# zhoujoey/ORB-SLAM3-Mac

Measured on AMD Instinct MI355X. Metric: ORB extract+match frames/sec, higher is better.
Workload: dtype u8; 1 GPU; vga: synthetic 640x480 batch=1024 per GPU, 8-level pyramid, 1000 feats/frame, ORB extract + Hamming 2-NN match (Frame.cc:1146) + SearchForInitialization (ORBmatcher.cc:710) vs successor frame; pipelines=1, matchers=side by side (two contexts), frames_total=1024

## Files before the change

### orb-slam3-mac_amd/csrc/orb_internal.h

```cpp
#pragma once
#include <hip/hip_runtime.h>
#include <stdint.h>
#include "../../include/orbhip.h"

#define ORB_MAX_LEVELS 16
#define ORB_EDGE 19
#define ORB_MINB 16
#define ORB_HALF_PATCH 15
#define ORB_RS_STEPS 24

struct OrbLevel {
    uint8_t *img;
    uint8_t *blur;
    size_t img_frame_stride;
    size_t blur_frame_stride;
    int w, h, img_pitch, blur_pitch;
    int ncols, nrows, wcell, hcell;
    int cell_base;
    int cell_cap;
    int quota;
    int key_base, key_cap;
    int kp_base, kp_cap;
    int n_ini;
    float hx;
    float scale;
    float size;
    const int16_t *xofs; const int16_t *xalpha; const int16_t *yofs; const int16_t *ybeta;
    const uint32_t *xchunk; const uint32_t *ytab;
    int resize_mode;
    int rs_rows;
};

struct OrbParams {
    OrbLevel lv[ORB_MAX_LEVELS];
    int nlevels, batch;
    int n_cus;
    int ini_th, min_th;
    int cells_per_frame;
    int keys_per_frame;
    int kps_per_frame;
    int max_kp;
    int oct_nc;
    int rows_min_batch;
    int bm_min_batch;
    int br_blocks[ORB_MAX_LEVELS + 1];
    int bs_tiles[ORB_MAX_LEVELS + 1];
    int lap0, lap1;
    uint32_t *cell_count;
    uint32_t *cell_list;
    size_t cell_list_frame_stride;
    uint32_t *keys;
    uint16_t *node_of;
    uint32_t *lvl_kp;
#define ORB_PERM_MIN_BATCH 16
    uint16_t *lvl_perm;
    float *lvl_angle;
    uint8_t *lvl_desc;
    int32_t *lvl_count;
    int32_t *lvl_ncand;
    int32_t *status;
    orbhip_keypoint *out_kp;
    uint8_t *out_desc;
    int32_t *out_count;
    int32_t *out_mono;
    int umax[ORB_HALF_PATCH + 1];
// ... 43 lines not shown
struct StereoArgs {
    StereoLevel lv[ORB_MAX_LEVELS];
    int nlevels, batch, max_kp, rows0;
    const orbhip_keypoint *kpL, *kpR;
    const uint8_t *descL, *descR;
    const int32_t *nL, *nR;
    float mb, mbf;
    float *u_right, *depth;
    int32_t *sad, *n_kept;
};
void orb_launch_stereo(const StereoArgs &A, hipStream_t s);

int orb_lds_optin(const void *func, int device, size_t need);

void orb_launch_resize(const OrbParams &P, int level, hipStream_t s);
void orb_launch_fast_cells(const FastParams &F, hipStream_t s, int max_per_cu, int lvl_lo = 0, int lvl_hi = -1);
const void *orb_fast_runs_func(int nld);
#define ORB_OVERLAP_MIN_BATCH 16
#ifndef BLR_R
#define BLR_R 24
#endif
void orb_launch_blur(const OrbParams &P, hipStream_t s, int wgs_per_cu, int frame0 = 0, int nframes = -1);
const void *orb_fast_cells_func(int small);
void orb_launch_octree(const OrbParams &P, hipStream_t s);
void orb_launch_orient_desc(const OrbParams &P, hipStream_t s);
void orb_launch_assemble(const OrbParams &P, hipStream_t s);
size_t orb_octree_lds_bytes(int nc);
int orb_octree_nc(const OrbParams &P);
const void *orb_octree_func();
```

### orb-slam3-mac_amd/csrc/orb_kernels.hip

```cpp
#include "orb_internal.h"
#include "wave_dpp.h"
#include <mutex>
#include <vector>
#include <cstdio>
#include <cstdlib>

#define WAVE 64

__device__ __forceinline__ int wave_incl_scan(int v) { return wave_scan_add_dpp(v); }

__device__ __forceinline__ int block_excl_scan256(int v, int *wsum, int *total)
{
    const int lane = threadIdx.x & (WAVE - 1), wid = threadIdx.x >> 6;
    int inc = wave_incl_scan(v);
    if (lane == WAVE - 1) wsum[wid] = inc;
    __syncthreads();
    int base = 0;
#pragma unroll
    for (int w = 0; w < 4; w++) {
        int s = wsum[w];
        if (w < wid) base += s;
    }
    *total = wsum[0] + wsum[1] + wsum[2] + wsum[3];
    __syncthreads();
// ... 784 lines not shown
}

__device__ __forceinline__ int oct_quadrant(uint32_t key, uint32_t b0, uint32_t b1)
{
    const int x0 = b0 & 0xFFFF, y0 = b0 >> 16, x1 = b1 & 0xFFFF, y1 = b1 >> 16;
    const int mx = x0 + ((x1 - x0 + 1) >> 1), my = y0 + ((y1 - y0 + 1) >> 1);
    const int kx = ORB_KEY_X(key), ky = ORB_KEY_Y(key);
    return (kx < mx ? 0 : 1) + (ky < my ? 0 : 2);
}

#define OCT_KR 8
#ifdef OCT_PROF
__device__ long long g_oct_prof[8];
#define OCT_T(i) do { if (blockIdx.x == 0 && threadIdx.x == 0) { const long long t_ = clock64(); g_oct_prof[i] += t_ - t_prev; t_prev = t_; } } while (0)
extern "C" int orbhip_debug_oct_prof(long long *out8, int reset)
{
    if (out8 && hipMemcpyFromSymbol(out8, HIP_SYMBOL(g_oct_prof), 64) != hipSuccess) return -1;
    if (reset) { long long z[8] = {0}; if (hipMemcpyToSymbol(HIP_SYMBOL(g_oct_prof), z, 64) != hipSuccess) return -1; }
    return 0;
}
#else
#define OCT_T(i) do { } while (0)
#endif
__global__ __launch_bounds__(256) void k_octree(OrbParams P)
{
    extern __shared__ uint32_t smem[];
    __shared__ int wsum[8];
    __shared__ int s_size, s_front, s_nexpand, s_rstar, s_T, s_nproc;
    const int tid = threadIdx.x;
#ifdef OCT_PROF
    long long t_prev = clock64();
#endif
    const int lvl = blockIdx.x / P.batch;
    const int frame = blockIdx.x - lvl * P.batch;
    const OrbLevel &L = P.lv[lvl];
    const int N = L.quota;
    const int NC = P.oct_nc;
    uint32_t *box0 = smem, *box1 = smem + NC, *cnt = smem + 2 * NC;
    uint32_t *nbox0 = smem + 3 * NC, *nbox1 = smem + 4 * NC, *ncnt = smem + 5 * NC;
    OctLds S;
    {
        uint32_t *p = smem + 6 * NC;
        S.cc = p; p += 4 * NC;
        S.ord = (int *)p; p += NC; S.by_ord = (int *)p; p += NC; S.excl = (int *)p; p += NC;
        S.posbase = (int *)p; p += NC; S.newpos = (int *)p; p += NC; S.best = p; p += NC;
    }
    const uint32_t *ccount = P.cell_count + (size_t)frame * P.cells_per_frame + L.cell_base;
    const uint32_t *clist = P.cell_list + (size_t)frame * P.cell_list_frame_stride + (size_t)L.cell_base * L.cell_cap;
    uint32_t *keys = P.keys + (size_t)frame * P.keys_per_frame + L.key_base;
    uint16_t *node_of = P.node_of + (size_t)frame * P.keys_per_frame + L.key_base;
    const int ncells = L.ncols * L.nrows;
    uint32_t rk[OCT_KR]; int rn[OCT_KR];
    int running = 0;
    int32_t *count_out = P.lvl_count + frame * P.nlevels + lvl;
    if (ncells + 1 <= 16 * NC) {
        int *coff = reinterpret_cast<int *>(smem);
        for (int c0 = 0; c0 < ncells; c0 += 256) {
            const int c = c0 + tid;
            const int n = c < ncells ? min((int)ccount[c], L.cell_cap) : 0;
            int total;
            const int off = running + block_excl_scan256(n, wsum, &total);
            if (c < ncells) coff[c] = off;
            running += total;
        }
        if (tid == 0) coff[ncells] = running;
        __syncthreads();
        if (running > L.key_cap) { if (tid == 0) atomicExch(P.status, ORBHIP_E_CAPACITY); running = L.key_cap; }
        const int K0 = running;
        auto fetch = [&](int k) {
            int lo = 0, hi = ncells;
            while (hi - lo > 1) { const int mid = (lo + hi) >> 1; if (coff[mid] <= k) lo = mid; else hi = mid; }
            return clist[(size_t)lo * L.cell_cap + (k - coff[lo])];
        };
#pragma unroll
        for (int i = 0; i < OCT_KR; i++) { const int k = tid + 256 * i; rk[i] = k < K0 ? fetch(k) : 0u; rn[i] = 0; }
#pragma unroll
        for (int i = 0; i < OCT_KR; i++) { const int k = tid + 256 * i; if (k < K0) keys[k] = rk[i]; }
        for (int k = tid + 256 * OCT_KR; k < K0; k += 256) keys[k] = fetch(k);
        __syncthreads();
    } else {
        for (int c0 = 0; c0 < ncells; c0 += 256) {
            const int c = c0 + tid;
            const int n = c < ncells ? (int)ccount[c] : 0;
            int total;
            const int off = running + block_excl_scan256(n, wsum, &total);
            for (int i = 0; i < n; i++)
                if (off + i < L.key_cap) keys[off + i] = clist[(size_t)c * L.cell_cap + i];
            running += total;
        }
        if (running > L.key_cap) { if (tid == 0) atomicExch(P.status, ORBHIP_E_CAPACITY); running = L.key_cap; }
        __syncthreads();
        __threadfence_block();
#pragma unroll
        for (int i = 0; i < OCT_KR; i++) { const int k = tid + 256 * i; rk[i] = k < running ? keys[k] : 0u; rn[i] = 0; }
    }
    const int K = running;
    if (tid == 0) P.lvl_ncand[frame * P.nlevels + lvl] = K;
    if (K == 0) { if (tid == 0) *count_out = 0; return; }
    __syncthreads();
    __threadfence_block();
    OCT_T(0);
    const int n_ini = L.n_ini;
    const int H = (L.h - ORB_MINB) - ORB_MINB;
    for (int i = tid; i < NC; i += 256) { cnt[i] = 0; ncnt[i] = 0; }
    __syncthreads();
#pragma unroll
    for (int i = 0; i < OCT_KR; i++)
        if (tid + 256 * i < K) {
            const int r = (int)__fdiv_rn((float)ORB_KEY_X(rk[i]), L.hx);
            rn[i] = r;
            atomicAdd(&ncnt[r], 1u);
        }
    for (int k = tid + 256 * OCT_KR; k < K; k += 256) {
        const int r = (int)__fdiv_rn((float)ORB_KEY_X(keys[k]), L.hx);
        node_of[k] = (uint16_t)r;
        atomicAdd(&ncnt[r], 1u);
    }
    __syncthreads();
    if (tid == 0) {
        int m = 0;
// ... 143 lines not shown
                int r = 0;
                for (int j = 3; j > qd; j--) r += q[j] > 0;
                return S.posbase[p] + r;
            }
            return S.newpos[p];
        };
#pragma unroll
        for (int i = 0; i < OCT_KR; i++) if (tid + 256 * i < K) rn[i] = relabel(rk[i], rn[i]);
        for (int k = tid + 256 * OCT_KR; k < K; k += 256) node_of[k] = (uint16_t)relabel(keys[k], node_of[k]);
        __syncthreads();
        const int new_size = T + (size - nproc);
        const int nexpand = s_nexpand;
        { uint32_t *t; t = box0; box0 = nbox0; nbox0 = t; t = box1; box1 = nbox1; nbox1 = t; t = cnt; cnt = ncnt; ncnt = t; }
        const int old_size = size;
        size = new_size; front = T;
#ifdef OCT_PROF
        if (blockIdx.x == 0 && tid == 0) g_oct_prof[5] += 1;
#endif
        if (new_size >= N || new_size == old_size) break;
        if (!final_phase && new_size + 3 * nexpand > N) final_phase = true;
    }
    __syncthreads();
    OCT_T(2);
    for (int i = tid; i < size; i += 256) S.best[i] = 0;
    __syncthreads();
#pragma unroll
    for (int i = 0; i < OCT_KR; i++)
        if (tid + 256 * i < K) atomicMax(&S.best[rn[i]], ((uint32_t)ORB_KEY_S(rk[i]) << 20) | (uint32_t)(0xFFFFF - (tid + 256 * i)));
    for (int k = tid + 256 * OCT_KR; k < K; k += 256)
        atomicMax(&S.best[node_of[k]], ((uint32_t)ORB_KEY_S(keys[k]) << 20) | (uint32_t)(0xFFFFF - k));
    __syncthreads();
    OCT_T(3);
    uint32_t *out = P.lvl_kp + (size_t)frame * P.kps_per_frame + L.kp_base;
    int nout = size;
    if (nout > L.kp_cap) { if (tid == 0) atomicExch(P.status, ORBHIP_E_CAPACITY); nout = L.kp_cap; }
    uint16_t *perm = P.lvl_perm + (size_t)frame * P.kps_per_frame + L.kp_base;
    for (int i = tid; i < nout; i += 256) out[i] = keys[0xFFFFF - (S.best[i] & 0xFFFFF)];
    if (P.batch < ORB_PERM_MIN_BATCH) { if (tid == 0) *count_out = nout; return; }
    __syncthreads();
    for (int i = tid; i < nout; i += 256) { const uint32_t ki = out[i]; S.best[i] = ((uint32_t)(ORB_KEY_Y(ki) >> 5) << 16) | (uint32_t)ORB_KEY_X(ki); }
    __syncthreads();
    for (int i = tid; i < nout; i += 256) {
        const uint32_t si = S.best[i];
        int rank = 0;
        for (int j = 0; j < nout; j++) { const uint32_t sj = S.best[j]; rank += (sj < si) || (sj == si && j < i); }
        perm[rank] = (uint16_t)i;
    }
    if (tid == 0) *count_out = nout;
    OCT_T(4);
}

const void *orb_octree_func() { return reinterpret_cast<const void *>(k_octree); }

void orb_launch_octree(const OrbParams &P, hipStream_t s)
{
    const size_t lds = orb_octree_lds_bytes(P.oct_nc);
    hipLaunchKernelGGL(k_octree, dim3(P.nlevels * P.batch), dim3(256), lds, s, P);
}

#define BL_TW 64
#define BL_TH 32
#define BL_ROWS (BL_TH + 6)
#define BL_IPD 20
__device__ __forceinline__ int reflect101(int p, int n)
{
    if (p < 0) p = -p;
    if (p >= n) p = 2 * n - 2 - p;
    return p;
}

__device__ __forceinline__ uint32_t bl_load4(const uint8_t *row, int x, int w)
{
    if (x >= 0 && x + 3 < w) return *reinterpret_cast<const uint32_t *>(row + x);
    uint32_t v = 0;
#pragma unroll
    for (int j = 0; j < 4; j++) {
        int xx = reflect101(x + j, w);
        xx = min(max(xx, 0), w - 1);
        v |= (uint32_t)row[xx] << (8 * j);
    }
// ... 579 lines not shown
```

### orb-slam3-mac_amd/csrc/orbhip_api.hip

```cpp
#include "orb_internal.h"
#include "ctx_internal.h"
#include <cmath>
#include <cfloat>
#include <cstdio>
#include <cstdlib>
#include <cstring>
#include <string>
#include <vector>
#include <mutex>
#include <set>
#include <utility>

static thread_local std::string g_last_error;
extern "C" const char *orbhip_last_error(void) { return g_last_error.c_str(); }
extern "C" const char *orbhip_version(void) { return "orbhip 0.1 (gfx950)"; }

#define HIP_TRY(expr)                                                                   \
    do {                                                                                \
        hipError_t _e = (expr);                                                         \
        if (_e != hipSuccess) {                                                         \
            g_last_error = std::string(#expr) + ": " + hipGetErrorString(_e);           \
            return ORBHIP_E_HIP;                                                        \
        }                                                                               \
    } while (0)
// ... 185 lines not shown
    int width, height, max_batch;
    bool level0_owned;
    OrbParams P;
    FastParams F;
    std::vector<void *> allocs;
    size_t bytes_reserved;
    int last_batch;
    bool profiling;
    hipEvent_t ev[ORBHIP_PROF_SLOTS][ORBHIP_STAGE_COUNT + 1];
    int ev_calls;
    bool ev_created;
    float stage_ms[ORBHIP_STAGE_COUNT];
    uint8_t *d_level0;
    int32_t *d_stereo_sad;
    bool graph_mode, graph_valid;
    hipStream_t aux; hipEvent_t ev_fork, ev_join, ev_pyr; bool aux_ok; int overlap;
    hipGraphExec_t graph_exec;
    int g_w, g_h, g_batch, g_lap0, g_lap1;
    size_t level0_frame_stride; int level0_pitch;
    uint8_t *d_outblob; size_t outblob_bytes, ob_kp, ob_desc;
    uint8_t *h_out; uint8_t *h_in; size_t h_in_bytes; int32_t *h_status;
    uint8_t *h_pyr; size_t h_pyr_bytes;
    unsigned long long generation, view_generation;
};

extern "C" int orbhip_extractor_create(orbhip_ctx *ctx, int nfeatures, float scale_factor, int nlevels,
                                       int ini_th, int min_th, orbhip_extractor **out)
{
    if (!ctx || !out || nlevels < 1 || nlevels > ORB_MAX_LEVELS || nfeatures < 1 || !(scale_factor > 1.0f) || scale_factor > 2.0f)
        return ORBHIP_E_BADARG;
    orbhip_extractor *e = new orbhip_extractor();
    e->ctx = ctx; e->nfeatures = nfeatures; e->nlevels = nlevels; e->ini_th = ini_th; e->min_th = min_th;
    e->scale_factor = scale_factor;
    e->width = e->height = e->max_batch = 0; e->bytes_reserved = 0; e->last_batch = 0;
    e->profiling = false; e->ev_created = false; e->ev_calls = 0; e->d_level0 = nullptr; e->level0_owned = false;
    e->d_stereo_sad = nullptr;
    e->graph_mode = false; e->graph_valid = false; e->graph_exec = nullptr;
    e->aux = nullptr; e->ev_fork = e->ev_join = e->ev_pyr = nullptr; e->aux_ok = false; e->overlap = 1;
    e->d_outblob = nullptr; e->outblob_bytes = e->ob_kp = e->ob_desc = 0; e->h_out = e->h_in = e->h_pyr = nullptr; e->h_in_bytes = e->h_pyr_bytes = 0; e->h_status = nullptr;
    e->generation = 0; e->view_generation = ~0ull;
    memset(&e->P, 0, sizeof(e->P));
    memset(e->stage_ms, 0, sizeof(e->stage_ms));
    e->scale[0] = 1.0f; e->sigma2[0] = 1.0f;
    for (int i = 1; i < nlevels; i++) { e->scale[i] = e->scale[i - 1] * scale_factor; e->sigma2[i] = e->scale[i] * e->scale[i]; }
    for (int i = 0; i < nlevels; i++) { e->inv_scale[i] = 1.0f / e->scale[i]; e->inv_sigma2[i] = 1.0f / e->sigma2[i]; }
    float factor = 1.0f / scale_factor;
// ... 338 lines not shown
    }
    if ((rc = dev_alloc(e, &P.cell_count, B * cells))) return rc;
    if ((rc = dev_alloc(e, &P.cell_list, B * P.cell_list_frame_stride))) return rc;
    if ((rc = dev_alloc(e, &P.keys, B * keys))) return rc;
    if ((rc = dev_alloc(e, &P.node_of, B * keys))) return rc;
    if ((rc = dev_alloc(e, &P.lvl_kp, B * kps))) return rc;
    if ((rc = dev_alloc(e, &P.lvl_perm, B * kps))) return rc;
    if ((rc = dev_alloc(e, &P.lvl_angle, B * kps))) return rc;
    if ((rc = dev_alloc(e, &P.lvl_desc, B * kps * 32))) return rc;
    if ((rc = dev_alloc(e, &P.lvl_count, B * e->nlevels))) return rc;
    if ((rc = dev_alloc(e, &P.lvl_ncand, B * e->nlevels))) return rc;
    if ((rc = dev_alloc(e, &P.status, 1))) return rc;
    {
        auto up = [](size_t v) { return (v + 255) & ~(size_t)255; };
        e->ob_kp = up(8 * B); e->ob_desc = e->ob_kp + up(sizeof(orbhip_keypoint) * B * P.max_kp);
        e->outblob_bytes = e->ob_desc + up((size_t)32 * B * P.max_kp);
        if ((rc = dev_alloc(e, &e->d_outblob, e->outblob_bytes))) return rc;
        P.out_count = reinterpret_cast<int32_t *>(e->d_outblob); P.out_mono = P.out_count + B;
        P.out_kp = reinterpret_cast<orbhip_keypoint *>(e->d_outblob + e->ob_kp); P.out_desc = e->d_outblob + e->ob_desc;
    }
    HIP_TRY(hipMemset(P.status, 0, sizeof(int32_t)));
    P.oct_nc = orb_octree_nc(P);
    if (orb_octree_lds_bytes(P.oct_nc) > 150 * 1024) { g_last_error = "per-level quota (or nIni) too large for the LDS-resident octree"; return ORBHIP_E_BADARG; }
    if ((rc = orb_lds_optin(orb_octree_func(), e->ctx->device, orb_octree_lds_bytes(P.oct_nc)))) return rc;
    if ((rc = orb_lds_optin(orb_fast_cells_func(e->F.small_cells), e->ctx->device, sizeof(uint32_t) * (size_t)e->F.wave_dw))) return rc;
    if (e->F.use_runs && (rc = orb_lds_optin(orb_fast_runs_func((e->F.run_rows - 7) * 5 <= 256 ? 4 : 6), e->ctx->device, sizeof(uint32_t) * (size_t)e->F.run_dw))) return rc;
    e->width = width; e->height = height; e->max_batch = max_batch;
    return ORBHIP_OK;
}

extern "C" int orbhip_compute_stereo_matches_device(orbhip_extractor *left, orbhip_extractor *right, float mb, float mbf,
                                                    float *d_u_right, float *d_depth, int32_t *d_n_matches)
{
    if (!left || !right || !d_u_right || !d_depth || !(mb > 0) || !(mbf > 0)) return ORBHIP_E_BADARG;
    if (!left->max_batch || !right->max_batch || left->last_batch <= 0 || left->last_batch != right->last_batch ||
        left->width != right->width || left->height != right->height || left->nlevels != right->nlevels ||
        left->scale_factor != right->scale_factor || left->P.max_kp != right->P.max_kp || left->P.max_kp > 65535) {
        g_last_error = "stereo: extractors must share geometry, feature budget and batch, and have extracted";
        return ORBHIP_E_BADARG;
    }
    HIP_TRY(hipSetDevice(left->ctx->device));
    if (!left->d_stereo_sad) {
        int rc = dev_alloc(left, &left->d_stereo_sad, (size_t)left->max_batch * left->P.max_kp);
        if (rc) return rc;
    }
    if (right->ctx->stream != left->ctx->stream) {
        hipEvent_t ev;
// ... 473 lines not shown
    return ORBHIP_OK;
}

extern "C" int orbhip_extractor_get_fast_candidates(orbhip_extractor *e, int frame, int level, int32_t *xs, int32_t *ys,
                                                    int32_t *scores, int cap, int32_t *n_out)
{
    if (!e || level < 0 || level >= e->nlevels || frame < 0 || frame >= e->last_batch || !n_out) return ORBHIP_E_BADARG;
    const OrbParams &P = e->P;
    const OrbLevel &L = P.lv[level];
    HIP_TRY(hipSetDevice(e->ctx->device));
    HIP_TRY(hipStreamSynchronize(e->ctx->stream));
    int32_t n = 0;
    HIP_TRY(hipMemcpy(&n, P.lvl_ncand + frame * P.nlevels + level, sizeof(n), hipMemcpyDeviceToHost));
    *n_out = n;
    int m = std::min(n, cap);
    if (m > 0 && xs && ys && scores) {
        std::vector<uint32_t> k(m);
        HIP_TRY(hipMemcpy(k.data(), P.keys + (size_t)frame * P.keys_per_frame + L.key_base, sizeof(uint32_t) * m, hipMemcpyDeviceToHost));
        for (int i = 0; i < m; i++) { xs[i] = ORB_KEY_X(k[i]); ys[i] = ORB_KEY_Y(k[i]); scores[i] = ORB_KEY_S(k[i]); }
    }
    return ORBHIP_OK;
}

extern "C" int orbhip_extractor_get_level_keypoints(orbhip_extractor *e, int frame, int level, orbhip_keypoint *out,
                                                    int cap, int32_t *n_out)
{
    if (!e || level < 0 || level >= e->nlevels || frame < 0 || frame >= e->last_batch || !n_out) return ORBHIP_E_BADARG;
    const OrbParams &P = e->P;
    const OrbLevel &L = P.lv[level];
    HIP_TRY(hipSetDevice(e->ctx->device));
    HIP_TRY(hipStreamSynchronize(e->ctx->stream));
    int32_t n = 0;
    HIP_TRY(hipMemcpy(&n, P.lvl_count + frame * P.nlevels + level, sizeof(n), hipMemcpyDeviceToHost));
    *n_out = n;
    int m = std::min(n, cap);
    if (m > 0 && out) {
        std::vector<uint32_t> k(m); std::vector<float> a(m);
        const size_t off = (size_t)frame * P.kps_per_frame + L.kp_base;
        HIP_TRY(hipMemcpy(k.data(), P.lvl_kp + off, sizeof(uint32_t) * m, hipMemcpyDeviceToHost));
        HIP_TRY(hipMemcpy(a.data(), P.lvl_angle + off, sizeof(float) * m, hipMemcpyDeviceToHost));
        for (int i = 0; i < m; i++) {
            out[i].x = (float)(ORB_KEY_X(k[i]) + ORB_MINB); out[i].y = (float)(ORB_KEY_Y(k[i]) + ORB_MINB);
            out[i].size = L.size; out[i].angle = a[i]; out[i].response = (float)ORB_KEY_S(k[i]);
            out[i].octave = level; out[i].class_id = -1;
        }
    }
// ... 3 lines not shown
```

### orb-slam3-mac_amd/python/orbhip.py

```python
import ctypes as C
import os
import numpy as np

try:
    import torch
except Exception:
    torch = None

_HERE = os.path.dirname(os.path.abspath(__file__))
LIB_DIR = os.path.join(os.path.dirname(_HERE), "lib")
LIB_PATH = os.path.join(LIB_DIR, "liborbhip.so")
SYNTH_PATH = os.path.join(LIB_DIR, "libsynth.so")

if not os.path.exists(LIB_PATH):
    raise ImportError(
        "liborbhip.so not built: run `python -c 'import __graft_entry__ as g; g.build()'` "
        "(there is no CPU fallback for the HIP path)")

lib = C.CDLL(LIB_PATH)

OK, E_BADARG, E_NODEVICE, E_HIP, E_CAPACITY, E_ABORTED, E_NOTSPD, E_EMPTY = 0, -1, -2, -3, -4, -5, -6, -7
STAGES = ["pyramid", "fast_cells", "blur", "octree", "desc", "assemble"]

KP_DTYPE = np.dtype([("x", "<f4"), ("y", "<f4"), ("size", "<f4"), ("angle", "<f4"),
# ... 18 lines not shown
lib.orbhip_extractor_max_keypoints.argtypes = [vp]
lib.orbhip_extract_batch_device.argtypes = [vp, vp, ci, ci, sz, sz, ci, ci, ci]
lib.orbhip_extractor_results.argtypes = [vp, C.POINTER(vp), C.POINTER(vp), C.POINTER(vp), C.POINTER(vp)]
lib.orbhip_extract_batch_host.argtypes = [vp, vp, ci, ci, sz, sz, ci, ci, ci, vp, vp, ci, vp, vp]
lib.orbhip_extractor_level_dims.argtypes = [vp, ci, C.POINTER(ci), C.POINTER(ci)]
lib.orbhip_extractor_get_pyramid_level.argtypes = [vp, ci, ci, ci, vp, sz]
lib.orbhip_extractor_get_blurred_level.argtypes = [vp, ci, ci, vp, sz]
lib.orbhip_extractor_get_pyramid_padded.argtypes = [vp, ci, vp, vp]
lib.orbhip_extractor_get_fast_candidates.argtypes = [vp, ci, ci, vp, vp, vp, ci, C.POINTER(C.c_int32)]
lib.orbhip_extractor_get_level_keypoints.argtypes = [vp, ci, ci, vp, ci, C.POINTER(C.c_int32)]
lib.orbhip_extractor_set_profiling.argtypes = [vp, ci]
lib.orbhip_extractor_set_graph_mode.argtypes = [vp, ci]
lib.orbhip_extractor_stage_ms.argtypes = [vp, vp]
lib.orbhip_descriptor_distance.argtypes = [vp, vp]
lib.orbhip_match_bf2nn_device.argtypes = [vp, vp, vp, sz, vp, vp, sz, ci, ci, cd, vp, vp, vp]
lib.orbhip_search_for_initialization_device.argtypes = [vp, vp, vp, vp, vp, vp, vp, ci, ci, sz, cf, cf, cf, cf, ci, cf, ci,
                                                        vp, vp, vp]
lib.orbhip_ctx_check_status.argtypes = [vp]
lib.orbhip_ctx_wait_for.argtypes = [vp, vp]
lib.orbhip_extractor_blur_kernel.argtypes = [vp, ci]
lib.orbhip_extractor_blur_kernel.restype = ci
lib.orbhip_extractor_resize_band_rows.argtypes = [vp, ci]
lib.orbhip_extractor_resize_band_rows.restype = ci
lib.orbhip_prev_matched_init_device.argtypes = [vp, vp, sz, ci, ci, vp]
lib.orbhip_search_by_projection_device.argtypes = [vp, vp, vp, vp, ci, vp, vp, vp, vp, ci, sz, ci, cf, cf, cf, cf, ci, ci, vp, vp]
lib.orbhip_search_local_map_device.argtypes = [vp, vp, vp, vp, ci, vp, vp, vp, vp, ci, sz, ci, cf, cf, cf, cf, ci, cf, vp, vp]


class OrbHipError(RuntimeError):
    def __init__(self, code, where):
        self.code = code
        super().__init__("%s failed: %d (%s)" % (where, code, lib.orbhip_last_error().decode()))


def _chk(rc, where):
    if rc != OK:
        raise OrbHipError(rc, where)


class Context:
    def __init__(self, device=0, stream=None):
        h = vp()
        _chk(lib.orbhip_ctx_create(device, stream, C.byref(h)), "orbhip_ctx_create")
        self.h = h

    def synchronize(self):
# ... 35 lines not shown

    def features_per_level(self):
        out = np.zeros(self.nlevels, np.int32)
        _chk(lib.orbhip_extractor_features_per_level(self.h, out.ctypes.data), "features_per_level")
        return out

    def umax(self):
        out = np.zeros(16, np.int32)
        _chk(lib.orbhip_extractor_umax(self.h, out.ctypes.data), "umax")
        return out

    def reserve(self, w, h, batch):
        _chk(lib.orbhip_extractor_reserve(self.h, w, h, batch), "orbhip_extractor_reserve")

    @property
    def max_keypoints(self):
        return lib.orbhip_extractor_max_keypoints(self.h)

    def blur_kernel(self, batch):
        return ("k_blur", "k_blur_rows", "k_blur_mfma")[lib.orbhip_extractor_blur_kernel(self.h, int(batch))]

    def resize_band_rows(self, level):
        return lib.orbhip_extractor_resize_band_rows(self.h, int(level))

    def set_graph_mode(self, on):
        _chk(lib.orbhip_extractor_set_graph_mode(self.h, 1 if on else 0), "orbhip_extractor_set_graph_mode")

    def set_profiling(self, on):
        _chk(lib.orbhip_extractor_set_profiling(self.h, 1 if on else 0), "set_profiling")

    def stage_ms(self):
        out = np.zeros(len(STAGES), np.float32)
        _chk(lib.orbhip_extractor_stage_ms(self.h, out.ctypes.data), "stage_ms")
        return dict(zip(STAGES, out.tolist()))

    def extract_host(self, images, lap=(0, 1000)):
        img = np.ascontiguousarray(images, np.uint8)
        if img.ndim == 2:
            img = img[None]
        B, H, W = img.shape
        self.reserve(W, H, B)
        cap = self.max_keypoints
        kp = np.zeros((B, cap), KP_DTYPE)
        desc = np.zeros((B, cap, 32), np.uint8)
        cnt = np.zeros(B, np.int32)
        mono = np.zeros(B, np.int32)
# ... 767 lines not shown
```

Measured before the change: 318,500 frames/s.

## Add table-based octree keypoint distribution with iterative fallback redo kernel

Adds a table form of the octree distribution. Each keypoint's quadtree path is computed directly to a fixed depth, counts are built bottom-up in LDS, and the stopping level is chosen from per-depth tallies instead of splitting nodes iteratively. Lists the table form cannot resolve are marked with count -1, and a second kernel reruns the original iterative octree on those lists only. This aims to cut the serial per-iteration split and scan work, at the cost of an extra launch, more LDS tables, and a more complex path that must stay consistent with the iterative semantics.

```diff
diff --git a/orb-slam3-mac_amd/csrc/orb_internal.h b/orb-slam3-mac_amd/csrc/orb_internal.h
--- a/orb-slam3-mac_amd/csrc/orb_internal.h
+++ b/orb-slam3-mac_amd/csrc/orb_internal.h
@@ -41,6 +41,7 @@
     int kps_per_frame;
     int max_kp;
     int oct_nc;
+    int oct_dmax;
     int rows_min_batch;
     int bm_min_batch;
     int br_blocks[ORB_MAX_LEVELS + 1];
@@ -130,9 +131,10 @@
 #endif
 void orb_launch_blur(const OrbParams &P, hipStream_t s, int wgs_per_cu, int frame0 = 0, int nframes = -1);
 const void *orb_fast_cells_func(int small);
-void orb_launch_octree(const OrbParams &P, hipStream_t s);
+void orb_launch_octree(const OrbParams &P, hipStream_t s, int parts = 3);
 void orb_launch_orient_desc(const OrbParams &P, hipStream_t s);
 void orb_launch_assemble(const OrbParams &P, hipStream_t s);
 size_t orb_octree_lds_bytes(int nc);
 int orb_octree_nc(const OrbParams &P);
-const void *orb_octree_func();
+int orb_octree_dmax(const OrbParams &P);
+const void *orb_octree_func(int which = 0);
diff --git a/orb-slam3-mac_amd/csrc/orb_kernels.hip b/orb-slam3-mac_amd/csrc/orb_kernels.hip
--- a/orb-slam3-mac_amd/csrc/orb_kernels.hip
+++ b/orb-slam3-mac_amd/csrc/orb_kernels.hip
@@ -830,17 +830,103 @@
 #else
 #define OCT_T(i) do { } while (0)
 #endif
-__global__ __launch_bounds__(256) void k_octree(OrbParams P)
+__device__ __forceinline__ int oct_gather(const OrbParams &P, const OrbLevel &L, int frame, int lvl, uint32_t *smem, int NC, int *wsum,
+                                          uint32_t (&rk)[OCT_KR], uint32_t *keys)
+{
+    const int tid = threadIdx.x;
+    const uint32_t *ccount = P.cell_count + (size_t)frame * P.cells_per_frame + L.cell_base;
+    const uint32_t *clist = P.cell_list + (size_t)frame * P.cell_list_frame_stride + (size_t)L.cell_base * L.cell_cap;
+    const int ncells = L.ncols * L.nrows;
+    int running = 0;
+    if (ncells + 1 <= 16 * NC) {
+        int *coff = reinterpret_cast<int *>(smem);
+        for (int c0 = 0; c0 < ncells; c0 += 256) {
+            const int c = c0 + tid;
+            const int n = c < ncells ? min((int)ccount[c], L.cell_cap) : 0;
+            int total;
+            const int off = running + block_excl_scan256(n, wsum, &total);
+            if (c < ncells) coff[c] = off;
+            running += total;
+        }
+        if (tid == 0) coff[ncells] = running;
+        __syncthreads();
+        if (running > L.key_cap) { if (tid == 0) atomicExch(P.status, ORBHIP_E_CAPACITY); running = L.key_cap; }
+        const int K0 = running;
+        auto fetch = [&](int k) {
+            int lo = 0, hi = ncells;
+            while (hi - lo > 1) { const int mid = (lo + hi) >> 1; if (coff[mid] <= k) lo = mid; else hi = mid; }
+            return clist[(size_t)lo * L.cell_cap + (k - coff[lo])];
+        };
+#pragma unroll
+        for (int i = 0; i < OCT_KR; i++) { const int k = tid + 256 * i; rk[i] = k < K0 ? fetch(k) : 0u; }
+#pragma unroll
+        for (int i = 0; i < OCT_KR; i++) { const int k = tid + 256 * i; if (k < K0) keys[k] = rk[i]; }
+        for (int k = tid + 256 * OCT_KR; k < K0; k += 256) keys[k] = fetch(k);
+        __syncthreads();
+    } else {
+        for (int c0 = 0; c0 < ncells; c0 += 256) {
+            const int c = c0 + tid;
+            const int n = c < ncells ? (int)ccount[c] : 0;
+            int total;
+            const int off = running + block_excl_scan256(n, wsum, &total);
+            for (int i = 0; i < n; i++)
+                if (off + i < L.key_cap) keys[off + i] = clist[(size_t)c * L.cell_cap + i];
+            running += total;
+        }
+        if (running > L.key_cap) { if (tid == 0) atomicExch(P.status, ORBHIP_E_CAPACITY); running = L.key_cap; }
+        __syncthreads();
+        __threadfence_block();
+#pragma unroll
+        for (int i = 0; i < OCT_KR; i++) { const int k = tid + 256 * i; rk[i] = k < running ? keys[k] : 0u; }
+    }
+    if (tid == 0) P.lvl_ncand[frame * P.nlevels + lvl] = running;
+    return running;
+}
+
+__device__ __forceinline__ void oct_output(const OrbParams &P, const OrbLevel &L, int frame, int lvl, uint32_t *best, int size, int K,
+                                           const uint32_t (&rk)[OCT_KR], const int (&rn)[OCT_KR], const uint32_t *keys, const uint16_t *node_of,
+                                           long long &t_prev)
+{
+    const int tid = threadIdx.x;
+    int32_t *count_out = P.lvl_count + frame * P.nlevels + lvl;
+    for (int i = tid; i < size; i += 256) best[i] = 0;
+    __syncthreads();
+#pragma unroll
+    for (int i = 0; i < OCT_KR; i++)
+        if (tid + 256 * i < K) atomicMax(&best[rn[i]], ((uint32_t)ORB_KEY_S(rk[i]) << 20) | (uint32_t)(0xFFFFF - (tid + 256 * i)));
+    for (int k = tid + 256 * OCT_KR; k < K; k += 256)
+        atomicMax(&best[node_of[k]], ((uint32_t)ORB_KEY_S(keys[k]) << 20) | (uint32_t)(0xFFFFF - k));
+    __syncthreads();
+    OCT_T(3);
+    uint32_t *out = P.lvl_kp + (size_t)frame * P.kps_per_frame + L.kp_base;
+    int nout = size;
+    if (nout > L.kp_cap) { if (tid == 0) atomicExch(P.status, ORBHIP_E_CAPACITY); nout = L.kp_cap; }
+    uint16_t *perm = P.lvl_perm + (size_t)frame * P.kps_per_frame + L.kp_base;
+    for (int i = tid; i < nout; i += 256) out[i] = keys[0xFFFFF - (best[i] & 0xFFFFF)];
+    if (P.batch < ORB_PERM_MIN_BATCH) { if (tid == 0) *count_out = nout; return; }
+    __syncthreads();
+    for (int i = tid; i < nout; i += 256) { const uint32_t ki = out[i]; best[i] = ((uint32_t)(ORB_KEY_Y(ki) >> 5) << 16) | (uint32_t)ORB_KEY_X(ki); }
+    __syncthreads();
+    for (int i = tid; i < nout; i += 256) {
+        const uint32_t si = best[i];
+        int rank = 0;
+        for (int j = 0; j < nout; j++) { const uint32_t sj = best[j]; rank += (sj < si) || (sj == si && j < i); }
+        perm[rank] = (uint16_t)i;
+    }
+    if (tid == 0) *count_out = nout;
+    OCT_T(4);
+}
+
+__device__ __forceinline__ void oct_iterative(const OrbParams &P, const int lvl, const int frame)
 {
     extern __shared__ uint32_t smem[];
     __shared__ int wsum[8];
     __shared__ int s_size, s_front, s_nexpand, s_rstar, s_T, s_nproc;
     const int tid = threadIdx.x;
+    long long t_prev = 0;
 #ifdef OCT_PROF
-    long long t_prev = clock64();
+    t_prev = clock64();
 #endif
-    const int lvl = blockIdx.x / P.batch;
-    const int frame = blockIdx.x - lvl * P.batch;
     const OrbLevel &L = P.lv[lvl];
     const int N = L.quota;
     const int NC = P.oct_nc;
@@ -853,57 +939,13 @@
         S.ord = (int *)p; p += NC; S.by_ord = (int *)p; p += NC; S.excl = (int *)p; p += NC;
         S.posbase = (int *)p; p += NC; S.newpos = (int *)p; p += NC; S.best = p; p += NC;
     }
-    const uint32_t *ccount = P.cell_count + (size_t)frame * P.cells_per_frame + L.cell_base;
-    const uint32_t *clist = P.cell_list + (size_t)frame * P.cell_list_frame_stride + (size_t)L.cell_base * L.cell_cap;
     uint32_t *keys = P.keys + (size_t)frame * P.keys_per_frame + L.key_base;
     uint16_t *node_of = P.node_of + (size_t)frame * P.keys_per_frame + L.key_base;
-    const int ncells = L.ncols * L.nrows;
     uint32_t rk[OCT_KR]; int rn[OCT_KR];
-    int running = 0;
     int32_t *count_out = P.lvl_count + frame * P.nlevels + lvl;
-    if (ncells + 1 <= 16 * NC) {
-        int *coff = reinterpret_cast<int *>(smem);
-        for (int c0 = 0; c0 < ncells; c0 += 256) {
-            const int c = c0 + tid;
-            const int n = c < ncells ? min((int)ccount[c], L.cell_cap) : 0;
-            int total;
-            const int off = running + block_excl_scan256(n, wsum, &total);
-            if (c < ncells) coff[c] = off;
-            running += total;
-        }
-        if (tid == 0) coff[ncells] = running;
-        __syncthreads();
-        if (running > L.key_cap) { if (tid == 0) atomicExch(P.status, ORBHIP_E_CAPACITY); running = L.key_cap; }
-        const int K0 = running;
-        auto fetch = [&](int k) {
-            int lo = 0, hi = ncells;
-            while (hi - lo > 1) { const int mid = (lo + hi) >> 1; if (coff[mid] <= k) lo = mid; else hi = mid; }
-            return clist[(size_t)lo * L.cell_cap + (k - coff[lo])];
-        };
-#pragma unroll
-        for (int i = 0; i < OCT_KR; i++) { const int k = tid + 256 * i; rk[i] = k < K0 ? fetch(k) : 0u; rn[i] = 0; }
-#pragma unroll
-        for (int i = 0; i < OCT_KR; i++) { const int k = tid + 256 * i; if (k < K0) keys[k] = rk[i]; }
-        for (int k = tid + 256 * OCT_KR; k < K0; k += 256) keys[k] = fetch(k);
-        __syncthreads();
-    } else {
-        for (int c0 = 0; c0 < ncells; c0 += 256) {
-            const int c = c0 + tid;
-            const int n = c < ncells ? (int)ccount[c] : 0;
-            int total;
-            const int off = running + block_excl_scan256(n, wsum, &total);
-            for (int i = 0; i < n; i++)
-                if (off + i < L.key_cap) keys[off + i] = clist[(size_t)c * L.cell_cap + i];
-            running += total;
-        }
-        if (running > L.key_cap) { if (tid == 0) atomicExch(P.status, ORBHIP_E_CAPACITY); running = L.key_cap; }
-        __syncthreads();
-        __threadfence_block();
-#pragma unroll
-        for (int i = 0; i < OCT_KR; i++) { const int k = tid + 256 * i; rk[i] = k < running ? keys[k] : 0u; rn[i] = 0; }
-    }
-    const int K = running;
-    if (tid == 0) P.lvl_ncand[frame * P.nlevels + lvl] = K;
+    const int K = oct_gather(P, L, frame, lvl, smem, NC, wsum, rk, keys);
+#pragma unroll
+    for (int i = 0; i < OCT_KR; i++) rn[i] = 0;
     if (K == 0) { if (tid == 0) *count_out = 0; return; }
     __syncthreads();
     __threadfence_block();
@@ -1093,40 +1135,272 @@
     }
     __syncthreads();
     OCT_T(2);
-    for (int i = tid; i < size; i += 256) S.best[i] = 0;
+    oct_output(P, L, frame, lvl, S.best, size, K, rk, rn, keys, node_of, t_prev);
+}
+
+__global__ __launch_bounds__(256) void k_octree(OrbParams P)
+{
+    const int lvl = blockIdx.x / P.batch;
+    oct_iterative(P, lvl, blockIdx.x - lvl * P.batch);
+}
+
+#define OCT_DMAX_LIMIT 7
+#define OCT_TAB_NODE_WORDS 9
+__host__ __device__ __forceinline__ int oct_tab_off(int n_ini, int d) { return n_ini * (((1 << (2 * d)) - 1) / 3); }
+
+int orb_octree_dmax(const OrbParams &P)
+{
+    int n_ini = 1;
+    for (int l = 0; l < P.nlevels; l++) n_ini = P.lv[l].n_ini > n_ini ? P.lv[l].n_ini : n_ini;
+    int d = 0;
+    while (d < OCT_DMAX_LIMIT && (long)oct_tab_off(n_ini, d + 2) <= (long)(16 - OCT_TAB_NODE_WORDS) * P.oct_nc) d++;
+    return d >= 2 ? d : 0;
+}
+
+__device__ __forceinline__ uint32_t oct_path(uint32_t key, const OrbLevel &L, int H, int D)
+{
+    const int kx = ORB_KEY_X(key), ky = ORB_KEY_Y(key);
+    const int r = min((int)__fdiv_rn((float)kx, L.hx), L.n_ini - 1);
+    int x0 = (int)__fmul_rn(L.hx, (float)r), x1 = (int)__fmul_rn(L.hx, (float)(r + 1)), y0 = 0, y1 = H;
+    uint32_t path = (uint32_t)r;
+    for (int d = 0; d < D; d++) {
+        const int mx = x0 + ((x1 - x0 + 1) >> 1), my = y0 + ((y1 - y0 + 1) >> 1);
+        const bool qx = kx >= mx, qy = ky >= my;
+        x0 = qx ? mx : x0; x1 = qx ? x1 : mx; y0 = qy ? my : y0; y1 = qy ? y1 : my;
+        path = (path << 2) | (uint32_t)((qx ? 1 : 0) + (qy ? 2 : 0));
+    }
+    return path;
+}
+
+__global__ __launch_bounds__(256) void k_octree_tab(OrbParams P)
+{
+    extern __shared__ uint32_t smem[];
+    __shared__ int wsum[8];
+    __shared__ int s_nz[OCT_DMAX_LIMIT + 1], s_mu[OCT_DMAX_LIMIT + 1];
+    __shared__ int s_front, s_rstar;
+    const int tid = threadIdx.x;
+    long long t_prev = 0;
+#ifdef OCT_PROF
+    t_prev = clock64();
+#endif
+    const int lvl = blockIdx.x / P.batch;
+    const int frame = blockIdx.x - lvl * P.batch;
+    const OrbLevel &L = P.lv[lvl];
+    const int N = L.quota, NC = P.oct_nc, D = P.oct_dmax, n_ini = L.n_ini;
+    const int H = (L.h - ORB_MINB) - ORB_MINB;
+    uint32_t *cnt = smem, *ncnt = smem + NC, *tix = smem + 2 * NC, *ntix = smem + 3 * NC;
+    int *ord = (int *)(smem + 4 * NC), *by_ord = (int *)(smem + 5 * NC), *excl = (int *)(smem + 6 * NC), *newpos = (int *)(smem + 7 * NC);
+    uint32_t *best = smem + 8 * NC, *tab = smem + OCT_TAB_NODE_WORDS * NC;
+    uint32_t *keys = P.keys + (size_t)frame * P.keys_per_frame + L.key_base;
+    uint16_t *node_of = P.node_of + (size_t)frame * P.keys_per_frame + L.key_base;
+    uint32_t rk[OCT_KR]; int rn[OCT_KR];
+    int32_t *count_out = P.lvl_count + frame * P.nlevels + lvl;
+    const int K = oct_gather(P, L, frame, lvl, smem, NC, wsum, rk, keys);
+    if (K == 0) { if (tid == 0) *count_out = 0; return; }
     __syncthreads();
-#pragma unroll
-    for (int i = 0; i < OCT_KR; i++)
-        if (tid + 256 * i < K) atomicMax(&S.best[rn[i]], ((uint32_t)ORB_KEY_S(rk[i]) << 20) | (uint32_t)(0xFFFFF - (tid + 256 * i)));
-    for (int k = tid + 256 * OCT_KR; k < K; k += 256)
-        atomicMax(&S.best[node_of[k]], ((uint32_t)ORB_KEY_S(keys[k]) << 20) | (uint32_t)(0xFFFFF - k));
+    OCT_T(0);
+    {
+        uint32_t *tabD = tab + oct_tab_off(n_ini, D);
+        for (int i = tid; i < (n_ini << (2 * D)); i += 256) tabD[i] = 0;
+        if (tid <= D) { s_nz[tid] = 0; s_mu[tid] = 0; }
+        __syncthreads();
+#pragma unroll
+        for (int i = 0; i < OCT_KR; i++) {
+            rn[i] = 0;
+            if (tid + 256 * i < K) { const uint32_t p = oct_path(rk[i], L, H, D); rn[i] = (int)p; atomicAdd(&tabD[p], 1u); }
+        }
+        for (int k = tid + 256 * OCT_KR; k < K; k += 256) atomicAdd(&tabD[oct_path(keys[k], L, H, D)], 1u);
+        __syncthreads();
+    }
+    for (int d = D; d >= 0; d--) {
+        uint32_t *t = tab + oct_tab_off(n_ini, d);
+        const uint32_t *c = tab + oct_tab_off(n_ini, d + 1);
+        int tally = 0;
+        for (int i = tid; i < (n_ini << (2 * d)); i += 256) {
+            uint32_t v;
+            if (d < D) { v = c[4 * i] + c[4 * i + 1] + c[4 * i + 2] + c[4 * i + 3]; t[i] = v; } else v = t[i];
+            tally += (v > 0 ? 1 : 0) + (v > 1 ? 0x10000 : 0);
+        }
+        tally = wave_sum_dpp(tally);
+        if ((tid & (WAVE - 1)) == 0 && tally) { atomicAdd(&s_nz[d], tally & 0xFFFF); atomicAdd(&s_mu[d], tally >> 16); }
+        __syncthreads();
+    }
+    OCT_T(1);
+    int T = 0;
+    bool final_phase = false;
+    {
+        int prev = s_nz[0];
+        for (int t = 1; t <= D; t++) {
+            const int sz = s_nz[t], nexpand = s_mu[t];
+            if (sz >= N || sz == prev) { T = t; break; }
+            if (sz + 3 * nexpand > N) { T = t; final_phase = true; break; }
+            if (nexpand == 0) { T = t; break; }
+            prev = sz;
+        }
+    }
+    if (T == 0) { if (tid == 0) *count_out = -1; return; }
+    int size, front, dcur = T;
+    {
+        const int E = oct_tab_off(n_ini, T + 1), per = (E + 255) >> 8;
+        const int e0 = min(tid * per, E), e1 = min(e0 + per, E);
+        auto entry = [&](int e, uint32_t &c, uint32_t &tx) {
+            int d = T, j = e;
+            while (j >= (n_ini << (2 * d))) { j -= n_ini << (2 * d); d--; }
+            const uint32_t m = (1u << (2 * d)) - 1;
+            int root = j >> (2 * d);
+            if (d & 1) root = n_ini - 1 - root;
+            const uint32_t raw = ((uint32_t)root << (2 * d)) | (((uint32_t)j & m) ^ (0x33333333u & m));
+            c = tab[oct_tab_off(n_ini, d) + raw];
+            tx = ((uint32_t)d << 27) | raw;
+            return c > 0 && (d == T || c == 1) && (d == 0 || tab[oct_tab_off(n_ini, d - 1) + (raw >> 2)] > 1);
+        };
+        uint32_t c, tx;
+        int nf = 0;
+        for (int e = e0; e < e1; e++) nf += entry(e, c, tx) ? 1 : 0;
+        int pos = block_excl_scan256(nf, wsum, &size);
+        if (size > NC) { if (tid == 0) *count_out = -1; return; }
+        for (int e = e0; e < e1; e++) {
+            if (e == (n_ini << (2 * T))) s_front = pos;
+            if (entry(e, c, tx)) { cnt[pos] = c; tix[pos] = tx; pos++; }
+        }
+        __syncthreads();
+        front = s_front;
+    }
+    while (final_phase) {
+        int C;
+        {
+            int run = 0;
+            for (int p0 = 0; p0 < size; p0 += 256) {
+                const int p = p0 + tid;
+                const int f = (p < front && cnt[p] > 1) ? 1 : 0;
+                int tot;
+                const int o = run + block_excl_scan256(f, wsum, &tot);
+                if (p < size) ord[p] = -1;
+                if (f) excl[o] = p;
+                run += tot;
+            }
+            C = run;
+        }
+        __syncthreads();
+        if (C == 0) break;
+        if (dcur == D) { if (tid == 0) *count_out = -1; return; }
+        for (int i = tid; i < C; i += 256) {
+            const int p = excl[i];
+            const uint32_t ci = cnt[p];
+            int r = 0;
+            for (int j = 0; j < C; j++) {
+                const uint32_t cj = cnt[excl[j]];
+                r += (cj > ci || (cj == ci && j < i)) ? 1 : 0;
+            }
+            ord[p] = r;
+            by_ord[r] = p;
+        }
+        if (tid == 0) s_rstar = C - 1;
+        __syncthreads();
+        const uint32_t *ctab = tab + oct_tab_off(n_ini, dcur + 1);
+        auto nchild = [&](int p) { const uint32_t *q = ctab + 4 * (tix[p] & 0x7FFFFFFu); return (q[0] > 0) + (q[1] > 0) + (q[2] > 0) + (q[3] > 0); };
+        {
+            int run = 0;
+            for (int o0 = 0; o0 < C; o0 += 256) {
+                const int o = o0 + tid;
+                const int nch = o < C ? nchild(by_ord[o]) : 0;
+                int tot;
+                const int e = run + block_excl_scan256(nch, wsum, &tot);
+                if (o < C) {
+                    excl[o] = e;
+                    if (size + e + nch - (o + 1) >= N) atomicMin(&s_rstar, o);
+                }
+                run += tot;
+            }
+        }
+        __syncthreads();
+        const int rstar = s_rstar;
+        const int Tn = excl[rstar] + nchild(by_ord[rstar]), nproc = rstar + 1;
+        {
+            int run = 0;
+            for (int p0 = 0; p0 < size; p0 += 256) {
+                const int p = p0 + tid;
+                const int surv = (p < size && !(ord[p] >= 0 && ord[p] <= rstar)) ? 1 : 0;
+                int tot;
+                const int e = run + block_excl_scan256(surv, wsum, &tot);
+                if (p < size && surv) newpos[p] = Tn + e;
+                run += tot;
+            }
+        }
+        for (int p = tid; p < size; p += 256) {
+            const int o = ord[p];
+            if (o >= 0 && o <= rstar) {
+                const uint32_t raw4 = 4 * (tix[p] & 0x7FFFFFFu);
+                const uint32_t *q = ctab + raw4;
+                int pos = Tn - (excl[o] + nchild(p));
+                for (int qd = 3; qd >= 0; qd--)
+                    if (q[qd]) { ncnt[pos] = q[qd]; ntix[pos] = ((uint32_t)(dcur + 1) << 27) | (raw4 + qd); pos++; }
+            } else {
+                const int np = newpos[p];
+                ncnt[np] = cnt[p]; ntix[np] = tix[p];
+            }
+        }
+        __syncthreads();
+        { uint32_t *t; t = cnt; cnt = ncnt; ncnt = t; t = tix; tix = ntix; ntix = t; }
+        const int old_size = size;
+        size = Tn + (size - nproc); front = Tn; dcur++;
+#ifdef OCT_PROF
+        if (blockIdx.x == 0 && tid == 0) g_oct_prof[5] += 1;
+#endif
+        if (size >= N || size == old_size) break;
+    }
+    {
+        const int Ef = oct_tab_off(n_ini, dcur + 1);
+        for (int i = tid; i < Ef; i += 256) tab[i] = 0xFFFFFFFFu;
+        __syncthreads();
+        for (int p = tid; p < size; p += 256) { const uint32_t tx = tix[p]; tab[oct_tab_off(n_ini, (int)(tx >> 27)) + (tx & 0x7FFFFFFu)] = (uint32_t)p; }
+        __syncthreads();
+        auto node = [&](uint32_t path) {
+            uint32_t nd = 0;
+            for (int d = 0; d <= dcur; d++) { const uint32_t v = tab[oct_tab_off(n_ini, d) + (path >> (2 * (D - d)))]; if (v != 0xFFFFFFFFu) nd = v; }
+            return (int)nd;
+        };
+#pragma unroll
+        for (int i = 0; i < OCT_KR; i++) if (tid + 256 * i < K) rn[i] = node((uint32_t)rn[i]);
+        for (int k = tid + 256 * OCT_KR; k < K; k += 256) node_of[k] = (uint16_t)node(oct_path(keys[k], L, H, D));
+    }
     __syncthreads();
-    OCT_T(3);
-    uint32_t *out = P.lvl_kp + (size_t)frame * P.kps_per_frame + L.kp_base;
-    int nout = size;
-    if (nout > L.kp_cap) { if (tid == 0) atomicExch(P.status, ORBHIP_E_CAPACITY); nout = L.kp_cap; }
-    uint16_t *perm = P.lvl_perm + (size_t)frame * P.kps_per_frame + L.kp_base;
-    for (int i = tid; i < nout; i += 256) out[i] = keys[0xFFFFF - (S.best[i] & 0xFFFFF)];
-    if (P.batch < ORB_PERM_MIN_BATCH) { if (tid == 0) *count_out = nout; return; }
+    OCT_T(2);
+    oct_output(P, L, frame, lvl, best, size, K, rk, rn, keys, node_of, t_prev);
+}
+
+__global__ __launch_bounds__(256) void k_octree_redo(OrbParams P)
+{
+    __shared__ unsigned long long s_todo;
+    const int tid = threadIdx.x, total = P.nlevels * P.batch, base = blockIdx.x * 64;
+    if (tid < 64) {
+        const int w = base + tid, lvl = w / P.batch;
+        const bool f = w < total && P.lvl_count[(w - lvl * P.batch) * P.nlevels + lvl] < 0;
+        const unsigned long long m = __ballot(f);
+        if (tid == 0) s_todo = m;
+    }
     __syncthreads();
-    for (int i = tid; i < nout; i += 256) { const uint32_t ki = out[i]; S.best[i] = ((uint32_t)(ORB_KEY_Y(ki) >> 5) << 16) | (uint32_t)ORB_KEY_X(ki); }
-    __syncthreads();
-    for (int i = tid; i < nout; i += 256) {
-        const uint32_t si = S.best[i];
-        int rank = 0;
-        for (int j = 0; j < nout; j++) { const uint32_t sj = S.best[j]; rank += (sj < si) || (sj == si && j < i); }
-        perm[rank] = (uint16_t)i;
-    }
-    if (tid == 0) *count_out = nout;
-    OCT_T(4);
-}
-
-const void *orb_octree_func() { return reinterpret_cast<const void *>(k_octree); }
-
-void orb_launch_octree(const OrbParams &P, hipStream_t s)
+    unsigned long long todo = s_todo;
+    while (todo) {
+        const int w = base + __ffsll((long long)todo) - 1, lvl = w / P.batch;
+        todo &= todo - 1;
+        oct_iterative(P, lvl, w - lvl * P.batch);
+        __syncthreads();
+    }
+}
+
+const void *orb_octree_func(int which)
+{
+    return which == 0 ? reinterpret_cast<const void *>(k_octree) : which == 1 ? reinterpret_cast<const void *>(k_octree_tab) : reinterpret_cast<const void *>(k_octree_redo);
+}
+
+void orb_launch_octree(const OrbParams &P, hipStream_t s, int parts)
 {
     const size_t lds = orb_octree_lds_bytes(P.oct_nc);
-    hipLaunchKernelGGL(k_octree, dim3(P.nlevels * P.batch), dim3(256), lds, s, P);
+    const int lists = P.nlevels * P.batch;
+    if (P.oct_dmax <= 0) { hipLaunchKernelGGL(k_octree, dim3(lists), dim3(256), lds, s, P); return; }
+    if (parts & 1) hipLaunchKernelGGL(k_octree_tab, dim3(lists), dim3(256), lds, s, P);
+    if (parts & 2) hipLaunchKernelGGL(k_octree_redo, dim3((lists + 63) / 64), dim3(256), lds, s, P);
 }
 
 #define BL_TW 64
diff --git a/orb-slam3-mac_amd/csrc/orbhip_api.hip b/orb-slam3-mac_amd/csrc/orbhip_api.hip
--- a/orb-slam3-mac_amd/csrc/orbhip_api.hip
+++ b/orb-slam3-mac_amd/csrc/orbhip_api.hip
@@ -231,6 +231,7 @@
     uint8_t *h_out; uint8_t *h_in; size_t h_in_bytes; int32_t *h_status;
     uint8_t *h_pyr; size_t h_pyr_bytes;
     unsigned long long generation, view_generation;
+    int oct_dmax_tab;
 };
 
 extern "C" int orbhip_extractor_create(orbhip_ctx *ctx, int nfeatures, float scale_factor, int nlevels,
@@ -615,7 +616,10 @@
     HIP_TRY(hipMemset(P.status, 0, sizeof(int32_t)));
     P.oct_nc = orb_octree_nc(P);
     if (orb_octree_lds_bytes(P.oct_nc) > 150 * 1024) { g_last_error = "per-level quota (or nIni) too large for the LDS-resident octree"; return ORBHIP_E_BADARG; }
-    if ((rc = orb_lds_optin(orb_octree_func(), e->ctx->device, orb_octree_lds_bytes(P.oct_nc)))) return rc;
+    for (int k = 0; k < 3; k++)
+        if ((rc = orb_lds_optin(orb_octree_func(k), e->ctx->device, orb_octree_lds_bytes(P.oct_nc)))) return rc;
+    e->oct_dmax_tab = orb_octree_dmax(P);
+    P.oct_dmax = getenv("ORBHIP_OCTREE") && !strcmp(getenv("ORBHIP_OCTREE"), "iterative") ? 0 : e->oct_dmax_tab;
     if ((rc = orb_lds_optin(orb_fast_cells_func(e->F.small_cells), e->ctx->device, sizeof(uint32_t) * (size_t)e->F.wave_dw))) return rc;
     if (e->F.use_runs && (rc = orb_lds_optin(orb_fast_runs_func((e->F.run_rows - 7) * 5 <= 256 ? 4 : 6), e->ctx->device, sizeof(uint32_t) * (size_t)e->F.run_dw))) return rc;
     e->width = width; e->height = height; e->max_batch = max_batch;
@@ -1135,6 +1139,57 @@
     return ORBHIP_OK;
 }
 
+extern "C" int orbhip_debug_octree(orbhip_extractor *e, int level, int nframes, const int32_t *offs, const int32_t *xs, const int32_t *ys,
+                                   const int32_t *scores, int form, uint32_t *out_keys, int cap, int32_t *out_counts, int32_t *out_redo)
+{
+    if (!e || !e->max_batch || level < 0 || level >= e->nlevels || nframes < 1 || nframes > e->max_batch || !offs || !out_keys || !out_counts ||
+        form < 0 || form > 1 || cap < 0) return ORBHIP_E_BADARG;
+    if (form == 1 && e->oct_dmax_tab <= 0) { g_last_error = "the table form of the octree cannot run at this geometry"; return ORBHIP_E_BADARG; }
+    OrbParams P = e->P;
+    const OrbLevel &L = P.lv[level];
+    P.batch = nframes; P.oct_dmax = form ? e->oct_dmax_tab : 0;
+    std::vector<uint32_t> count((size_t)nframes * P.cells_per_frame, 0), list((size_t)nframes * P.cell_list_frame_stride, 0);
+    for (int f = 0; f < nframes; f++) {
+        if (offs[f + 1] < offs[f] || offs[f + 1] - offs[f] > L.key_cap) return ORBHIP_E_CAPACITY;
+        for (int i = offs[f]; i < offs[f + 1]; i++) {
+            if (xs[i] < 0 || xs[i] >= L.w - 2 * ORB_MINB || ys[i] < 0 || ys[i] >= L.h - 2 * ORB_MINB || scores[i] < 0 || scores[i] > 255) return ORBHIP_E_BADARG;
+            const int c = std::min(ys[i] / L.hcell, L.nrows - 1) * L.ncols + std::min(xs[i] / L.wcell, L.ncols - 1);
+            uint32_t &n = count[(size_t)f * P.cells_per_frame + L.cell_base + c];
+            if ((int)n >= L.cell_cap) return ORBHIP_E_CAPACITY;
+            list[(size_t)f * P.cell_list_frame_stride + ((size_t)L.cell_base + c) * L.cell_cap + n++] = ORB_PACK_KEY(xs[i], ys[i], scores[i]);
+        }
+    }
+    HIP_TRY(hipSetDevice(e->ctx->device));
+    hipStream_t s = e->ctx->stream;
+    HIP_TRY(hipStreamSynchronize(s));
+    HIP_TRY(hipMemcpy(P.cell_count, count.data(), sizeof(uint32_t) * count.size(), hipMemcpyHostToDevice));
+    HIP_TRY(hipMemcpy(P.cell_list, list.data(), sizeof(uint32_t) * list.size(), hipMemcpyHostToDevice));
+    std::vector<int32_t> cnt((size_t)nframes * P.nlevels);
+    orb_launch_octree(P, s, 1);
+    HIP_TRY(hipGetLastError());
+    HIP_TRY(hipStreamSynchronize(s));
+    if (out_redo) {
+        HIP_TRY(hipMemcpy(cnt.data(), P.lvl_count, sizeof(int32_t) * cnt.size(), hipMemcpyDeviceToHost));
+        for (int f = 0; f < nframes; f++) out_redo[f] = cnt[(size_t)f * P.nlevels + level] < 0 ? 1 : 0;
+    }
+    if (form) orb_launch_octree(P, s, 2);
+    HIP_TRY(hipGetLastError());
+    HIP_TRY(hipStreamSynchronize(s));
+    HIP_TRY(hipMemcpy(cnt.data(), P.lvl_count, sizeof(int32_t) * cnt.size(), hipMemcpyDeviceToHost));
+    int32_t st = 0;
+    HIP_TRY(hipMemcpy(&st, P.status, sizeof(st), hipMemcpyDeviceToHost));
+    if (st) { HIP_TRY(hipMemset(P.status, 0, sizeof(int32_t))); return st; }
+    for (int f = 0; f < nframes; f++) {
+        const int n = cnt[(size_t)f * P.nlevels + level];
+        out_counts[f] = n;
+        if (n < 0) return ORBHIP_E_HIP;
+        const int m = std::min(n, cap);
+        if (m > 0) HIP_TRY(hipMemcpy(out_keys + (size_t)f * cap, P.lvl_kp + (size_t)f * P.kps_per_frame + L.kp_base, sizeof(uint32_t) * m, hipMemcpyDeviceToHost));
+    }
+    e->last_batch = 0;
+    return ORBHIP_OK;
+}
+
 extern "C" int orbhip_extractor_get_level_keypoints(orbhip_extractor *e, int frame, int level, orbhip_keypoint *out,
                                                     int cap, int32_t *n_out)
 {
diff --git a/orb-slam3-mac_amd/python/orbhip.py b/orb-slam3-mac_amd/python/orbhip.py
--- a/orb-slam3-mac_amd/python/orbhip.py
+++ b/orb-slam3-mac_amd/python/orbhip.py
@@ -64,6 +64,8 @@
 lib.orbhip_extractor_blur_kernel.restype = ci
 lib.orbhip_extractor_resize_band_rows.argtypes = [vp, ci]
 lib.orbhip_extractor_resize_band_rows.restype = ci
+if hasattr(lib, "orbhip_debug_octree"):
+    lib.orbhip_debug_octree.argtypes = [vp, ci, ci, vp, vp, vp, vp, ci, vp, ci, vp, vp]
 lib.orbhip_prev_matched_init_device.argtypes = [vp, vp, sz, ci, ci, vp]
 lib.orbhip_search_by_projection_device.argtypes = [vp, vp, vp, vp, ci, vp, vp, vp, vp, ci, sz, ci, cf, cf, cf, cf, ci, ci, vp, vp]
 lib.orbhip_search_local_map_device.argtypes = [vp, vp, vp, vp, ci, vp, vp, vp, vp, ci, sz, ci, cf, cf, cf, cf, ci, cf, vp, vp]
@@ -145,6 +147,19 @@
 
     def resize_band_rows(self, level):
         return lib.orbhip_extractor_resize_band_rows(self.h, int(level))
+
+    def debug_octree(self, level, lists, form):
+        offs = np.zeros(len(lists) + 1, np.int32)
+        offs[1:] = np.cumsum([len(l[0]) for l in lists])
+        xs, ys, ss = (np.ascontiguousarray(np.concatenate([np.asarray(l[k], np.int32) for l in lists] + [np.zeros(1, np.int32)])) for k in range(3))
+        cap = int(max(len(l[0]) for l in lists)) + 16
+        keys = np.zeros((len(lists), cap), np.uint32)
+        counts, redo = np.zeros(len(lists), np.int32), np.zeros(len(lists), np.int32)
+        _chk(lib.orbhip_debug_octree(self.h, int(level), len(lists), offs.ctypes.data, xs.ctypes.data, ys.ctypes.data, ss.ctypes.data,
+                                     {"iterative": 0, "table": 1}[form], keys.ctypes.data, cap, counts.ctypes.data, redo.ctypes.data),
+             "orbhip_debug_octree")
+        kept = [np.stack([k & 0xFFF, (k >> 12) & 0xFFF, k >> 24], 1).astype(np.int32) for k in (keys[f, :counts[f]] for f in range(len(lists)))]
+        return kept, redo.tolist()
 
     def set_graph_mode(self, on):
         _chk(lib.orbhip_extractor_set_graph_mode(self.h, 1 if on else 0), "orbhip_extractor_set_graph_mode")
```

After: 326,800 frames/s, median of 6. 1.03x the previous value.
